# CraigIDent/SpliSER

Measured on AMD Instinct MI355X. Metric: splice sites/sec (+ reads/sec) processed, higher is better.
Workload: dtype int32/u32 counters, f64 SSE

## Files before the change

spliser_amd/csrc/spl_device.h:

```cpp
#ifndef SPL_DEVICE_H
#define SPL_DEVICE_H

#include <stdint.h>
#include <hip/hip_vector_types.h>

#include "spl_pack.h"
#include "spl_devpack.h"

#ifndef SPL_BLOCK
#define SPL_BLOCK 256
#endif
#define SPL_COUNTER_STRIDE 64
#define SPL_WAVES (SPL_BLOCK / 64)
#ifndef SPL_K_SIMPLE
#define SPL_K_SIMPLE 4
#define SPL_K_MNM 2
#endif
#ifndef SPL_LIST_K
#define SPL_LIST_K 2
#endif
#ifndef SPL_WAVE_ITERS
#define SPL_WAVE_ITERS 10
#endif
#define SPL_WAVE_READS (64 * SPL_WAVE_ITERS)
#define SPL_TILE_FUSED_SHIFT 10
#define SPL_TILE_FUSED (1 << SPL_TILE_FUSED_SHIFT)
#define SPL_BLOCK_FUSED 256
#define SPL_WAVE_READS_FUSED 512
#define SPL_WIN 1020
#define SPL_WIN_STRANDED 956
#define SPL_WIN_STRANDED_FUSED 508
#define SPL_SERIAL_MAX 8
#ifndef SPL_AGG_ROUNDS
#define SPL_AGG_ROUNDS 2
#endif
#define SPL_LITERAL_WAVES 8192
#ifndef SPL_SCAN_BLOCK
#define SPL_SCAN_BLOCK 256
#endif


#define SPL_DEV_ERR_RANGE 1
#define SPL_DEV_ERR_TABLE 2

#define SPL_JF_COUNT_MASK 0x00ffffffu
#define SPL_JF_COMPLEX 0x40000000u
#define SPL_JF_MULTIROW 0x80000000u

#define SPL_SF_PLUS 1u
#define SPL_SF_MINUS 2u

struct spl_dbk {
    uint32_t first;
    uint32_t occ;
    uint32_t rival;
};

struct spl_count_params {
    int64_t n_reads;
    uint32_t n_chunks;
    const spl_chunk_meta *chunk_meta;
// ... 127 lines not shown
```

spliser_amd/csrc/spl_kernels.hip:

```cpp
#include <hip/hip_runtime.h>
#include <hip/hip_ext.h>
#include <cstdio>
#include <cstdlib>
#include <stdint.h>

#define SPL_HD __device__ __forceinline__
#include "spl_classify.h"
#include "spl_device.h"
#include "spl_layout_tile.h"

namespace {

__device__ __forceinline__ int32_t first_site_at_or_after(const spl_count_params &p, int32_t pos)
{
    const int64_t rel = (int64_t)pos - (int64_t)p.bucket_base;
    uint32_t b = 0;
    if (rel > 0) {
        const int64_t q = rel >> p.bucket_shift;
        b = q >= (int64_t)p.n_buckets ? p.n_buckets : (uint32_t)q;
    }
    uint32_t lo = p.bucket[b];
    uint32_t hi = p.bucket[b < p.n_buckets ? b + 1 : b];
    while (lo < hi) {
        const uint32_t mid = (lo + hi) >> 1;
// ... 328 lines not shown
    rv = (e.rival >> ((uint32_t)(x - p.dbase) & 31u)) & 1u;
}

typedef __attribute__((address_space(3))) int32_t spl_lds_i32;

template <int NARR, int WIN = (NARR == 4 ? SPL_WIN_STRANDED : SPL_WIN)>
__device__ __forceinline__ void commit_key(const spl_hot_params &p, spl_lds_i32 *lds, int32_t wbase, bool valid, uint32_t key, int32_t sign)
{
    if (valid) {
        const int arr = (int)(key & 3u);
        const int32_t d = (int32_t)(key >> 2);
        const uint32_t loc = (uint32_t)(d - wbase);
        if (loc <= (uint32_t)WIN) __hip_atomic_fetch_add(lds + (arr * (WIN + 1) + (int)loc), sign, __ATOMIC_RELAXED, __HIP_MEMORY_SCOPE_WORKGROUP);
        else atomicAdd(&p.diff[(int64_t)arr * p.diff_stride + d], sign);
    }
}

template <int NARR, int WIN>
__device__ __forceinline__ void commit_range(const spl_hot_params &p, spl_lds_i32 *lds, int32_t wbase, bool em, int32_t lo, int32_t ub, uint32_t arr)
{
    const uint32_t a = (uint32_t)(lo - wbase), b = (uint32_t)(ub - wbase);
    const bool inside = a <= (uint32_t)WIN && b <= (uint32_t)WIN;
    if (em && inside) {
        spl_lds_i32 *const row = lds + (int)arr * (WIN + 1);
        __hip_atomic_fetch_add(row + (int)a, 1, __ATOMIC_RELAXED, __HIP_MEMORY_SCOPE_WORKGROUP);
        __hip_atomic_fetch_add(row + (int)b, -1, __ATOMIC_RELAXED, __HIP_MEMORY_SCOPE_WORKGROUP);
    }
    if (__any(em && !inside)) {
        commit_key<NARR, WIN>(p, lds, wbase, em && !inside, ((uint32_t)lo << 2) | arr, 1);
        commit_key<NARR, WIN>(p, lds, wbase, em && !inside, ((uint32_t)ub << 2) | arr, -1);
    }
}

__device__ __forceinline__ void agg_add(uint32_t *addr, int32_t delta)
{
    const int lane = (int)__builtin_amdgcn_mbcnt_hi(~0u, __builtin_amdgcn_mbcnt_lo(~0u, 0u));
    unsigned long long todo = __ballot(1);
    const uint32_t lo = (uint32_t)(uintptr_t)addr, hi = (uint32_t)((uintptr_t)addr >> 32);
    for (int round = 0; round < SPL_AGG_ROUNDS; ++round) {
        const int leader = __ffsll((long long)todo) - 1;
        const bool same = (__shfl((int)lo, leader) == (int)lo) && (__shfl((int)hi, leader) == (int)hi);
        const unsigned long long grp = __ballot(same);
        const unsigned long long plus = __ballot(same && delta > 0);
        if (lane == leader) {
            const int32_t sum = 2 * (int32_t)__popcll(plus) - (int32_t)__popcll(grp);
            if (sum) atomicAdd(addr, (uint32_t)sum);
        }
        if (same) return;
        todo &= ~grp;
    }
    atomicAdd(addr, (uint32_t)delta);
}


__device__ __forceinline__ uint32_t junction_hash(int32_t l, int32_t r)
{
    uint32_t h = (uint32_t)l * 0x9E3779B1u ^ (uint32_t)r * 0x85EBCA77u;
    return h ^ (h >> 15);
}

template <bool STRANDED, int NARR, int WIN = (NARR == 4 ? SPL_WIN_STRANDED : SPL_WIN)>
__device__ __forceinline__ bool rivals_inline_from(const spl_hot_params &p, spl_lds_i32 *lds, int32_t wbase, int32_t l, int32_t r, uint32_t h,
                                                   uint4 ent, uint4 first, const int32_t *blk_a, const int32_t *blk_b, uint32_t sidx)
{
    bool found = false;
    for (int probe = 0; probe < 8; ++probe) {
// ... 92 lines not shown
                if (t > jl[a] && t < jr[a]) inside = a;
                if (jl[a] == t) { pu = jr[a]; alpha = true; }
                if (jr[a] == t) { pu = jl[a]; alpha = true; }
            }
#pragma unroll
            for (int b = 0; b < 3; ++b) cov |= (blk_a[b] <= t) && (t + 1 <= blk_b[b]);
            const bool beta1type = !alpha && inside < 0 && cov && strand_ok;
            if (alpha || beta1type) {
                const uint4 rx = p.jrivals[2u * (r_off[j] + i) + 1u];
                for (uint32_t e2 = 0; e2 < rx.z; ++e2) {
                    const int32_t pp = p.part_pos[rx.y + e2];
                    const bool is_end = pp == jl[0] || pp == jr[0] || pp == jl[1] || pp == jr[1];
                    if (is_end && !(alpha && pp == pu)) agg_add(&p.dbl[rx.y + e2], 1);
                }
                if (beta1type) {
                    commit_key<NARR, WIN>(p, lds, wbase, true, (td << 2) | a_b1, -1);
                    commit_key<NARR, WIN>(p, lds, wbase, true, ((td + 1u) << 2) | a_b1, 1);
                    commit_key<NARR, WIN>(p, lds, wbase, true, (td << 2) | a_me, 1);
                    commit_key<NARR, WIN>(p, lds, wbase, true, ((td + 1u) << 2) | a_me, -1);
                }
            } else if (inside >= j && strand_ok) {
                commit_key<NARR, WIN>(p, lds, wbase, true, (td << 2) | a_me, -1);
                commit_key<NARR, WIN>(p, lds, wbase, true, ((td + 1u) << 2) | a_me, 1);
            }
        }
    }
    return true;
}

}


template <bool STRANDED, bool BIG, bool FUSED>
__global__ __launch_bounds__(FUSED ? SPL_BLOCK_FUSED : SPL_BLOCK) __attribute__((amdgpu_waves_per_eu(FUSED ? 4 : 8, 8))) void spl_count_ranges_kernel(const spl_hot_params p)
{
    constexpr int NARR = STRANDED ? 4 : 2;
    constexpr int WIN = STRANDED ? (FUSED ? SPL_WIN_STRANDED_FUSED : SPL_WIN_STRANDED) : SPL_WIN;
    __shared__ int32_t lds_words[NARR * (WIN + 1)];
    spl_lds_i32 *const lds = (spl_lds_i32 *)lds_words;
    constexpr int BLOCK = FUSED ? SPL_BLOCK_FUSED : SPL_BLOCK, NWAVE = BLOCK / 64;
    constexpr int RPT = (int)SPL_TILE_FUSED / SPL_BLOCK_FUSED;
    constexpr uint32_t SEG = FUSED ? SPL_WAVE_READS_FUSED : SPL_WAVE_READS;
    constexpr uint32_t CSHIFT = BIG ? SPL_CHUNK_BIG_SHIFT : SPL_CHUNK_SHIFT;
    constexpr uint32_t TILE = SPL_TILE_FUSED, TILES = FUSED ? (1u << CSHIFT) / TILE : 1u;
    constexpr uint32_t REC_BYTES = FUSED ? (uint32_t)SPL_LAYOUT_SLOT(TILE) : 16u;
    __shared__ uint4 s_rec[REC_BYTES / 16u];
    __shared__ uint16_t s_idx[FUSED ? TILE : 1];
    __shared__ uint32_t s_lay[2 * NWAVE];
    typedef __attribute__((address_space(3))) const char spl_lchar;
    spl_lchar *const lrec = (spl_lchar *)s_rec;
    __shared__ uint16_t s_q[NWAVE * SEG];
    __shared__ uint32_t s_qcnt[NWAVE], s_qbase;
    const uint32_t wave = (uint32_t)__builtin_amdgcn_readfirstlane((int)(threadIdx.x >> 6));
    const uint32_t seg0 = wave * SEG;
    const uint32_t lane = (uint32_t)threadIdx.x & 63u;
    uint32_t n_front = 0, n_back = 0, back_done = 0;
    uint32_t fm_mnm = 0, it_mnm = 0;
    auto rank_in = [](unsigned long long m) {
        return (uint32_t)__builtin_amdgcn_mbcnt_hi((uint32_t)(m >> 32), __builtin_amdgcn_mbcnt_lo((uint32_t)m, 0u));
    };
    const uint32_t chunk_slot = my_chunk();
    const uint32_t ordered = chunk_slot < p.n_chunks ? p.chunk_order[chunk_slot] : 0xffffffffu;
    const bool live = ordered != 0xffffffffu;
    const uint32_t chunk = live ? ordered : 0u;
    uint32_t n_simple = 0;
    auto entry_of = [&](uint32_t slot) { return FUSED ? (uint32_t)((__attribute__((address_space(3))) const uint16_t *)s_idx)[(slot & 0x3fffu) - n_simple] : slot; };
    auto push_direct = [&](bool want, uint32_t slot, unsigned long long m, uint32_t n) {
        const uint32_t shard = blockIdx.x & 7u;
        uint32_t base = 0;
        if (lane == 0) base = atomicAdd(&p.queue_n[shard * SPL_COUNTER_STRIDE], n);
        base = (uint32_t)__builtin_amdgcn_readfirstlane((int)base);
        if (want) p.queue[(size_t)shard * p.queue_cap + base + rank_in(m)] = (chunk << CSHIFT) | entry_of(slot);
    };
    auto push_front = [&](bool want, uint32_t slot) {
        const unsigned long long m = __ballot(want);
        const uint32_t n = (uint32_t)__popcll(m);
        if (n_front + n_back - back_done + n > SEG) { push_direct(want, slot, m, n); return; }
        if (want) s_q[seg0 + n_front + rank_in(m)] = (uint16_t)entry_of(slot);
        n_front += n;
    };
    auto push_back = [&](bool want, uint32_t slot) {
        const unsigned long long m = __ballot(want);
        const uint32_t n = (uint32_t)__popcll(m);
        if (n_front + n_back + n > SEG) { push_front(want, slot & 0x3fffu); return; }
        if (want) s_q[seg0 + SEG - 1u - n_back - rank_in(m)] = (uint16_t)slot;
        n_back += n;
    };

    const int tid = threadIdx.x;
    int32_t wbase = 0;
    ChunkView cv;
    typedef __attribute__((address_space(1))) const uint32_t spl_gdw;
    auto dbk_at = [&](uint32_t s) { return (spl_gdw *)((__attribute__((address_space(1))) const char *)p.dbucket + (size_t)((s << 3) + (s << 2))); };
    auto dbk2 = [&](uint32_t s) { spl_gdw *q = dbk_at(s); spl_dbk e; e.first = q[0]; e.occ = q[1]; e.rival = 0u; return e; };
    auto dbk3 = [&](uint32_t s) { spl_gdw *q = dbk_at(s); spl_dbk e; e.first = q[0]; e.occ = q[1]; e.rival = q[2]; return e; };
    spl_layout_chunk ch;
    uint32_t tile = 0, tile_last = 0;
    uint32_t ob[TILES + 1];
    auto span_of = [&](uint32_t k) {
        const int64_t g0 = ch.lo & ~(int64_t)((1u << CSHIFT) - 1u), hi = ch.lo + ch.n;
        spllay::TileSpan sp;
        sp.cell0 = g0 + (int64_t)k * TILE;
        sp.lo = sp.cell0 > ch.lo ? sp.cell0 : ch.lo;
        sp.hi = sp.cell0 + TILE < hi ? sp.cell0 + TILE : hi;
        uint32_t a = ob[0], b = ob[1];
#pragma unroll
        for (uint32_t q = 1; q < TILES; ++q) { a = k == q ? ob[q] : a; b = k == q ? ob[q + 1] : b; }
        sp.o_lo = a; sp.o_hi = b; sp.o_fetch_hi = ch.o_hi; sp.seg_op0 = ch.seg_op0;
        return sp;
    };
    if constexpr (FUSED) {
        if (!live) return;
        ch = p.cells[chunk];
        const int64_t g0 = ch.lo & ~(int64_t)((1u << CSHIFT) - 1u), hi = ch.lo + ch.n;
        tile = (uint32_t)((ch.lo - g0) >> SPL_TILE_FUSED_SHIFT);
        tile_last = (uint32_t)((hi - 1 - g0) >> SPL_TILE_FUSED_SHIFT);
        const int32_t fp0 = p.src.pos[ch.lo] + ch.shift;
        const spl_dbk e_first = p.dbucket[dbk_slot(p, fp0 - 1)];
#pragma unroll
        for (uint32_t q = 0; q <= TILES; ++q) {
            int64_t i = g0 + (int64_t)q * TILE;
            i = i < ch.lo ? ch.lo : (i > hi ? hi : i);
            ob[q] = q == 0u ? ch.o_lo : (q == TILES ? ch.o_hi : p.src.cig_off[i]);
        }
        for (int j = tid; j < NARR * (WIN + 1); j += BLOCK) lds[j] = 0;
        cv.rec = nullptr;
        cv.wide = (spl_gu32 *)(p.src.cigar + ch.seg_op0);
        cv.shift = ch.shift;
        cv.first_pos = fp0 - ch.shift;
        { uint32_t nv; dbk_resolve(p, fp0 - 1, e_first, wbase, nv); }
    } else {
        cv = chunk_view(p.chunk_meta + chunk);
    }
    typedef uint32_t u32x4_a8 __attribute__((ext_vector_type(4), aligned(8)));
    auto ld_r4 = [&](uint32_t at) {
        if constexpr (FUSED) { const u32x4_a8 v = *(__attribute__((address_space(3))) const u32x4_a8 *)(lrec + at); return make_uint4(v.x, v.y, v.z, v.w); }
        else return ld_g4(cv.rec + (size_t)at);
    };
    auto ld_r2 = [&](uint32_t at) {
        if constexpr (FUSED) { const spl_u32x2 v = *(__attribute__((address_space(3))) const spl_u32x2 *)(lrec + at); return make_uint2(v.x, v.y); }
        else return ld_g2(cv.rec + (size_t)at);
    };
    for (;;) {
    if constexpr (FUSED) {
        const spllay::TileSpan sp = span_of(tile);
        uint32_t n[4];
        {
            spllay::TileLoads<(int)TILE, RPT> L;
            spllay::tile_issue<(int)TILE, RPT>(p.src, p.src_n_rec, p.src_n_ops, sp, L);
            spllay::tile_finish<(int)TILE, RPT>(p.src, p.src_n_ops, sp, L, (spllay::lay_lds_w32 *)s_rec, (spllay::lay_lds_w32 *)s_lay,
                                                spllay::RecordsInLds{(spllay::lay_lds_u8 *)s_rec, (spllay::lay_lds_u16 *)s_idx, tile * TILE}, n);
        }
        cv.start[0] = 0; cv.start[1] = n[0]; cv.start[2] = n[0] + n[1]; cv.start[3] = n[0] + n[1] + n[2]; cv.start[4] = n[0] + n[1] + n[2] + n[3];
        cv.off[0] = 0;
        cv.off[1] = (n[0] * SPL_REC_SIMPLE + 15u) & ~15u;
        cv.off[2] = cv.off[1] + n[1] * SPL_REC_MNM;
        cv.off[3] = cv.off[2] + n[2] * SPL_REC_M2;
        n_simple = n[0];
        __syncthreads();
    }
    constexpr uint32_t KS = SPL_K_SIMPLE, KM = SPL_K_MNM;
    uint32_t g_start[SPL_RC_RUNS + 1];
    g_start[0] = 0;
    g_start[1] = (cv.start[1] + 64u * KS - 1u) / (64u * KS);
    g_start[2] = g_start[1] + (cv.start[2] - cv.start[1] + 64u * KM - 1u) / (64u * KM);
    g_start[3] = g_start[2] + ((cv.start[3] - cv.start[2] + 63u) >> 6);
    g_start[4] = g_start[3] + ((cv.start[4] - cv.start[3] + 63u) >> 6);
    const uint32_t g_total = live ? g_start[SPL_RC_RUNS] : 0u;
    typedef uint4 W4;
    W4 cu0 = make_uint4(0, 0, 0, 0), cu1 = make_uint4(0, 0, 0, 0);
    uint32_t cu_i0 = 0;
    auto fetch = [&](uint32_t g) {
        const uint32_t run = (g >= g_start[1] ? 1u : 0u) + (g >= g_start[2] ? 1u : 0u) + (g >= g_start[3] ? 1u : 0u);
        uint32_t gs = 0, n_run = cv.start[1], off = 0, size = SPL_REC_SIMPLE, per = KS;
        if (run == 1u) { gs = g_start[1]; n_run = cv.start[2] - cv.start[1]; off = cv.off[1]; size = SPL_REC_MNM; per = KM; }
        if (run == 2u) { gs = g_start[2]; n_run = cv.start[3] - cv.start[2]; off = cv.off[2]; size = SPL_REC_M2; per = 1u; }
        if (run == 3u) { gs = g_start[3]; n_run = cv.start[4] - cv.start[3]; off = cv.off[3]; size = SPL_REC_OTHER; per = 1u; }
        const uint32_t i0 = (((g - gs) << 6) + lane) * per;

        cu_i0 = i0;
        const uint32_t r = off + (i0 < n_run ? i0 : 0u) * size;
        cu0 = ld_r4(r);
        cu1 = ld_r4(r + 16u);
    };
    if constexpr (!FUSED) { if (wave < g_total) fetch(wave); }
    if constexpr (!FUSED) {
        { const int32_t fp = cv.first_pos + cv.shift; uint32_t nv; const spl_dbk e = p.dbucket[dbk_slot(p, fp - 1)]; dbk_resolve(p, fp - 1, e, wbase, nv); }
        for (int j = tid; j < NARR * (WIN + 1); j += BLOCK) lds[j] = 0;
        __syncthreads();
    }

    {
        uint32_t g = live ? wave : g_start[SPL_RC_RUNS];
        auto fetch_next = [&]() { if constexpr (!FUSED) fetch(g + NWAVE < g_total ? g + NWAVE : g); };
        auto take = [&](uint32_t gs, uint32_t n_run, uint32_t off, uint32_t size, uint32_t per) {
            if constexpr (FUSED) {
                const uint32_t i0 = (((g - gs) << 6) + lane) * per;
                cu_i0 = i0;
                const uint32_t r = off + (i0 < n_run ? i0 : 0u) * size;
                cu0 = ld_r4(r);
                cu1 = ld_r4(r + 16u);
            }
        };
        for (; g < g_start[1]; g += NWAVE) {
            take(0u, cv.start[1], 0u, SPL_REC_SIMPLE, KS);
            const uint32_t i0 = cu_i0;
            const W4 r0 = cu0, r1 = cu1;
            const uint32_t n_run = cv.start[1];
            const uint32_t w[8] = {r0.x, r0.y, r0.z, r0.w, r1.x, r1.y, r1.z, r1.w};
            int32_t pos[KS], c1[KS];
            spl_dbk e0[KS], e1[KS];
#pragma unroll
            for (uint32_t j = 0; j < KS; ++j) {
                pos[j] = (int32_t)w[2 * j] + cv.shift;
                c1[j] = pos[j] + (int32_t)(w[2 * j + 1] >> 16);
                e0[j] = dbk2(dbk_slot(p, pos[j] - 1));
                e1[j] = dbk2(dbk_slot(p, c1[j] - 1));
            }
            fetch_next();
#pragma unroll
            for (uint32_t j = 0; j < KS; ++j) {
                int32_t ua, ub; uint32_t nva, nvb;
                dbk_resolve(p, pos[j] - 1, e0[j], ua, nva);
                dbk_resolve(p, c1[j] - 1, e1[j], ub, nvb);
                const int32_t lo = ua + (int32_t)nva;
                const bool emit = i0 + j < n_run && ub > lo;
                uint32_t arr = 0;
                if (STRANDED) arr = (spl_read_strand(w[2 * j + 1] & 0xffffu, p.stranded) == (uint8_t)'-') ? 1u : 0u;
                if (__any(emit)) commit_range<NARR, WIN>(p, lds, wbase, emit, lo, ub, arr);
            }
        }
        for (; g < g_start[2]; g += NWAVE) {
            take(g_start[1], cv.start[2] - cv.start[1], cv.off[1], SPL_REC_MNM, KM);
            const uint32_t i0 = cu_i0;
            const W4 r0 = cu0, r1 = cu1;
            const uint32_t n_run = cv.start[2] - cv.start[1];
// ... 209 lines not shown
                bool live[KM], undecided[KM];
                int32_t pos[KM], c0[KM], c1[KM], c2[KM];
                uint32_t h[KM];
                uint4 ent[KM], first[KM];
#pragma unroll
                for (uint32_t k = 0; k < KM; ++k) {
                    live[k] = ((bits >> k) & 1u) != 0u;
                    undecided[k] = false;
                    pos[k] = (int32_t)w[4 * k] + cv.shift;
                    c0[k] = pos[k] + (int32_t)(w[4 * k + 1] >> 16); c1[k] = c0[k] + (int32_t)w[4 * k + 2]; c2[k] = c1[k] + (int32_t)w[4 * k + 3];
                    h[k] = junction_hash(c0[k] - 1, c1[k] - 1);
                    ent[k] = first[k] = make_uint4(0x80000000u, 0u, 0u, 0u);
                    if (live[k]) {
                        const uint4 *hslot = p.jhash + 2u * (h[k] & p.jhash_mask);
                        ent[k] = hslot[0];
                        first[k] = hslot[1];
                    }
                }
#pragma unroll
                for (uint32_t k = 0; k < KM; ++k) {
                    uint32_t sidx = 0;
                    if (STRANDED) sidx = (spl_read_strand(w[4 * k + 1] & 0xffffu, p.stranded) == (uint8_t)'-') ? 1u : 0u;
                    const int32_t blk_a[2] = {pos[k], c1[k]}, blk_b[2] = {c0[k] - 1, c2[k] - 1};
                    if (live[k]) undecided[k] = !rivals_inline_from<STRANDED, NARR, WIN>(p, lds, wbase, c0[k] - 1, c1[k] - 1, h[k], ent[k], first[k], blk_a, blk_b, sidx);
                }
#pragma unroll
                for (uint32_t k = 0; k < KM; ++k)
                    if (__any(undecided[k])) push_front(undecided[k], cv.start[1] + i0 + k);
            }
        }
    }
    if constexpr (!FUSED) break;
    else {
        if (tile == tile_last) break;
        ++tile;
        fm_mnm = 0; it_mnm = 0; n_back = 0; back_done = 0;
        __syncthreads();
    }
    }
    if ((tid & 63) == 0) s_qcnt[tid >> 6] = n_front;
    __syncthreads();
    uint32_t q_start[NWAVE + 1];
    q_start[0] = 0;
#pragma unroll
    for (int w = 0; w < NWAVE; ++w) q_start[w + 1] = q_start[w] + s_qcnt[w];
    const uint32_t qn = q_start[NWAVE];
    if (qn) {
        const uint32_t shard = blockIdx.x & 7u;
        if (tid == 0) s_qbase = atomicAdd(&p.queue_n[shard * SPL_COUNTER_STRIDE], qn);
        __syncthreads();
        uint32_t *dst = p.queue + (size_t)shard * p.queue_cap + s_qbase;
        const uint32_t first = chunk << CSHIFT;
        for (uint32_t j = tid; j < qn; j += BLOCK) {
            uint32_t w = 0;
#pragma unroll
            for (int k = 1; k < NWAVE; ++k) w += (j >= q_start[k]) ? 1u : 0u;
            uint32_t base = 0;
#pragma unroll
            for (int k = 0; k < NWAVE; ++k) base = (w == (uint32_t)k) ? q_start[k] : base;
            dst[j] = first | (uint32_t)s_q[w * SEG + (j - base)];
        }
    }
    for (int j = tid; j < NARR * (WIN + 1); j += BLOCK) {
        const int32_t v = lds[j];
        if (v) {
            const int arr = j / (WIN + 1), loc = j - arr * (WIN + 1);
            atomicAdd(&p.diff[(int64_t)arr * p.diff_stride + wbase + loc], v);
        }
    }
}

namespace {
// ... 474 lines not shown
                       n_dpos, flag_pos, n_flag, dbase, n_dbuckets, out);
    return (int)hipGetLastError();
}

extern "C" int spl_dev_launch_clear(void *region, size_t bytes, void *stream)
{
    const size_t n16 = bytes / 16;
    size_t blocks = (n16 + 256 * 4 - 1) / (256 * 4);
    blocks = blocks < 1 ? 1 : (blocks > 4096 ? 4096 : blocks);
    hipLaunchKernelGGL(spl_clear_kernel, dim3((uint32_t)blocks), dim3(256), 0, (hipStream_t)stream, (uint4 *)region, n16);
    return (int)hipGetLastError();
}

extern "C" int spl_dev_launch_count(const spl_count_params *p, const spl_hot_params *h, int pairs, void *stream, int *grid_out, int *lds_out,
                                    void *ev_start, void *ev_stop)
{
    *grid_out = 0;
    *lds_out = 0;
    if (p->n_reads <= 0 || p->n_sites <= 0) return 0;
    const uint32_t slots = pairs ? ((p->n_chunks + 7u) / 8u) * 8u : h->n_chunks;
    const uint32_t grid = slots;
    *grid_out = (int)grid;
    hipStream_t st = (hipStream_t)stream;
    hipEvent_t e0 = (hipEvent_t)ev_start, e1 = (hipEvent_t)ev_stop;
    if (pairs) {
        *lds_out = 2 * SPL_WIN * 4 + SPL_BLOCK * 5 * 4 + 4;
        if (p->stranded) hipExtLaunchKernelGGL(spl_count_pairs_kernel<true>, dim3(grid), dim3(SPL_BLOCK), 0, st, e0, e1, 0, *p);
        else hipExtLaunchKernelGGL(spl_count_pairs_kernel<false>, dim3(grid), dim3(SPL_BLOCK), 0, st, e0, e1, 0, *p);
    } else {
        const bool big = h->chunk_shift == SPL_CHUNK_BIG_SHIFT;
        *lds_out = (p->stranded ? 4 * ((h->cells ? SPL_WIN_STRANDED_FUSED : SPL_WIN_STRANDED) + 1) : 2 * (SPL_WIN + 1)) * 4 + SPL_WAVES * SPL_WAVE_READS * 2 + 4 * SPL_WAVES + 4;
#define SPL_LAUNCH_RANGES(S, B) hipExtLaunchKernelGGL((spl_count_ranges_kernel<S, B, false>), dim3(grid), dim3(SPL_BLOCK), 0, st, e0, e1, 0, *h)
        if (h->cells) {
            *lds_out += (int)SPL_LAYOUT_SLOT(SPL_TILE_FUSED) + 2 * SPL_TILE_FUSED + (SPL_BLOCK_FUSED / 64) * SPL_WAVE_READS_FUSED * 2 - SPL_WAVES * SPL_WAVE_READS * 2;
#define SPL_LAUNCH_FUSED(S, B) hipExtLaunchKernelGGL((spl_count_ranges_kernel<S, B, true>), dim3(grid), dim3(SPL_BLOCK_FUSED), 0, st, e0, e1, 0, *h)
            if (p->stranded) { if (big) SPL_LAUNCH_FUSED(true, true); else SPL_LAUNCH_FUSED(true, false); }
            else { if (big) SPL_LAUNCH_FUSED(false, true); else SPL_LAUNCH_FUSED(false, false); }
#undef SPL_LAUNCH_FUSED
        } else if (p->stranded) {
            if (big) SPL_LAUNCH_RANGES(true, true); else SPL_LAUNCH_RANGES(true, false);
        } else {
            if (big) SPL_LAUNCH_RANGES(false, true); else SPL_LAUNCH_RANGES(false, false);
        }
#undef SPL_LAUNCH_RANGES
    }
    return (int)hipGetLastError();
}

extern "C" int spl_dev_launch_literal(const spl_count_params *p, const spl_queue_params *q, void *stream)
{
    if (p->n_reads <= 0 || p->n_sites <= 0) return 0;
    hipStream_t st = (hipStream_t)stream;
    const uint32_t grid = SPL_LITERAL_WAVES;
    if (p->stranded) hipLaunchKernelGGL(spl_count_literal_kernel<true>, dim3(grid), dim3(64), 0, st, *p, *q);
    else hipLaunchKernelGGL(spl_count_literal_kernel<false>, dim3(grid), dim3(64), 0, st, *p, *q);
    return (int)hipGetLastError();
}

extern "C" int spl_dev_launch_scan(const spl_scan_params *p, void *stream)
{
    if (p->n_dpos <= 0) return 0;
    hipStream_t st = (hipStream_t)stream;
    hipLaunchKernelGGL(spl_scan_apply_kernel, dim3(p->n_blocks), dim3(256), 0, st, *p);
    return (int)hipGetLastError();
}

extern "C" int spl_dev_launch_sse(const spl_sse_params *p, void *stream)
// ... 7 lines not shown
```

spliser_amd/csrc/spl_layout_tile.h:

```cpp
#ifndef SPL_LAYOUT_TILE_H
#define SPL_LAYOUT_TILE_H
#include <hip/hip_runtime.h>
#include <stdint.h>

#include "spl_pack.h"
#include "spl_devpack.h"

namespace spllay {

typedef uint32_t lay_u32x2 __attribute__((ext_vector_type(2)));
typedef uint32_t lay_u32x4 __attribute__((ext_vector_type(4)));
typedef lay_u32x2 lay_u32x2_a4 __attribute__((aligned(4)));
typedef lay_u32x4 lay_u32x4_a8 __attribute__((aligned(8)));
typedef __attribute__((address_space(3))) uint32_t lay_lds_w32;
typedef __attribute__((address_space(3))) int32_t lay_lds_i32;
typedef __attribute__((address_space(3))) uint8_t lay_lds_u8;
typedef __attribute__((address_space(3))) uint16_t lay_lds_u16;

typedef __attribute__((address_space(3))) const uint32_t lay_lds_u32;
struct StagedOps {
    static constexpr bool padded = true;
    lay_lds_u32 *p;
    __device__ __forceinline__ uint32_t operator()(uint32_t k) const { return p[k]; }
};
__device__ __forceinline__ uint32_t row_scan(uint32_t v)
{
    v += (uint32_t)__builtin_amdgcn_update_dpp(0, (int)v, 0x111, 0xf, 0xf, false);
    v += (uint32_t)__builtin_amdgcn_update_dpp(0, (int)v, 0x112, 0xf, 0xf, false);
    v += (uint32_t)__builtin_amdgcn_update_dpp(0, (int)v, 0x114, 0xf, 0xf, false);
    v += (uint32_t)__builtin_amdgcn_update_dpp(0, (int)v, 0x118, 0xf, 0xf, false);
    return v;
}

__device__ __forceinline__ uint32_t wave_scan(uint32_t v)
{
    v += (uint32_t)__builtin_amdgcn_update_dpp(0, (int)v, 0x111, 0xf, 0xf, false);
    v += (uint32_t)__builtin_amdgcn_update_dpp(0, (int)v, 0x112, 0xf, 0xf, false);
    v += (uint32_t)__builtin_amdgcn_update_dpp(0, (int)v, 0x114, 0xf, 0xf, false);
    v += (uint32_t)__builtin_amdgcn_update_dpp(0, (int)v, 0x118, 0xf, 0xf, false);
    v += (uint32_t)__builtin_amdgcn_update_dpp(0, (int)v, 0x142, 0xa, 0xf, false);
    v += (uint32_t)__builtin_amdgcn_update_dpp(0, (int)v, 0x143, 0xc, 0xf, false);
    return v;
}


struct RecordsInMemory {
    static constexpr bool wants_index = false;
    static constexpr bool clip_tier = false;
    uint8_t *rec_base;
    size_t slot_bytes;
    __device__ __forceinline__ uint8_t *rec() const { return rec_base + (size_t)blockIdx.x * slot_bytes; }
    __device__ __forceinline__ void st2(uint32_t d, lay_u32x2 v) const { *(lay_u32x2 *)(rec() + d) = v; }
    __device__ __forceinline__ void st4(uint32_t d, lay_u32x4 v) const { *(lay_u32x4_a8 *)(rec() + d) = v; }
    __device__ __forceinline__ void index(uint32_t, uint32_t) const {}
};
struct RecordsInLds {
    static constexpr bool wants_index = true;
    static constexpr bool clip_tier = true;
    lay_lds_u8 *rec;
    lay_lds_u16 *idx;
    uint32_t base;
    __device__ __forceinline__ void st2(uint32_t d, lay_u32x2 v) const { *(__attribute__((address_space(3))) lay_u32x2 *)(rec + d) = v; }
    __device__ __forceinline__ void st4(uint32_t d, lay_u32x4 v) const { *(__attribute__((address_space(3))) lay_u32x4_a8 *)(rec + d) = v; }
    __device__ __forceinline__ void index(uint32_t q, uint32_t cell_index) const { idx[q] = (uint16_t)(base + cell_index); }
};

struct TileSpan { int64_t cell0, lo, hi; uint32_t o_lo, o_hi, o_fetch_hi, seg_op0; };
template <int C, int R>
struct TileLoads {
    int32_t pos[R];
    uint32_t fw[R / 2];
    uint32_t co[R + 1];
    lay_u32x4 v[R];
};

template <int C, int R>
__device__ __forceinline__ void tile_issue(const spl_devreads &src, int64_t n_rec, int64_t n_ops, const TileSpan &sp, TileLoads<C, R> &L)
{
    static_assert(R == 4 || R == 2, "two or four reads a thread");
    constexpr uint32_t T = C / R, STAGE = 4 * C;
    static_assert(STAGE / (4 * T) == R, "R quads of ops a thread");
    const uint32_t t = threadIdx.x;
    const int64_t g = sp.cell0 + R * (int64_t)t;
#pragma unroll
    for (int j = 0; j < R; ++j) L.pos[j] = 0;
#pragma unroll
    for (int j = 0; j <= R; ++j) L.co[j] = 0;
#pragma unroll
    for (int j = 0; j < R / 2; ++j) L.fw[j] = 0;
    const uint32_t r0 = (uint32_t)R * t, lo_r = (uint32_t)(sp.lo - sp.cell0), hi_r = (uint32_t)(sp.hi - sp.cell0);
    const int64_t left = n_rec - sp.cell0;
    const uint32_t rec_r = left < (int64_t)C ? (uint32_t)left : (uint32_t)C;
    const bool mine = r0 + R > lo_r && r0 < hi_r;
    if (mine) {
        if (r0 + R <= rec_r) {
            if constexpr (R == 4) {
                const lay_u32x4 pv = *(const lay_u32x4 *)(src.pos + g);
                const lay_u32x2 fv = *(const lay_u32x2 *)(src.flag + g);
                const lay_u32x4 cv = *(const lay_u32x4 *)(src.cig_off + g);
                L.co[4] = src.cig_off[g + 4];
                L.pos[0] = (int32_t)pv.x; L.pos[1] = (int32_t)pv.y; L.pos[2] = (int32_t)pv.z; L.pos[3] = (int32_t)pv.w;
                L.fw[0] = fv.x; L.fw[1] = fv.y;
                L.co[0] = cv.x; L.co[1] = cv.y; L.co[2] = cv.z; L.co[3] = cv.w;
            } else {
                const lay_u32x2 pv = *(const lay_u32x2 *)(src.pos + g);
                L.fw[0] = *(const uint32_t *)(src.flag + g);
                const lay_u32x2 cv = *(const lay_u32x2 *)(src.cig_off + g);
                L.co[2] = src.cig_off[g + 2];
                L.pos[0] = (int32_t)pv.x; L.pos[1] = (int32_t)pv.y;
                L.co[0] = cv.x; L.co[1] = cv.y;
            }
        } else {
            uint32_t f[R];
#pragma unroll
            for (int j = 0; j < R; ++j) {
                const int64_t i = g + j;
                f[j] = 0;
                if (i < n_rec) { L.pos[j] = src.pos[i]; f[j] = src.flag[i]; L.co[j] = src.cig_off[i]; L.co[j + 1] = src.cig_off[i + 1]; }
                else L.co[j + 1] = L.co[j];
            }
#pragma unroll
            for (int j = 0; j < R / 2; ++j) L.fw[j] = f[2 * j] | (f[2 * j + 1] << 16);
        }
    }
    const uint64_t ws = sp.o_lo & ~3u;
    const uint64_t o_end = (uint64_t)sp.o_fetch_hi < ws + STAGE ? (uint64_t)sp.o_fetch_hi : ws + STAGE;
#pragma unroll
    for (uint32_t q = 0; q < (uint32_t)R; ++q) {
        const uint64_t at = ws + 4ull * (t + q * T);
        L.v[q] = lay_u32x4{0u, 0u, 0u, 0u};
        if (at < o_end) {
            if (at + 4 <= (uint64_t)n_ops) L.v[q] = *(const lay_u32x4 *)(src.cigar + at);
            else {
                L.v[q].x = src.cigar[at];
                if (at + 1 < (uint64_t)n_ops) L.v[q].y = src.cigar[at + 1];
                if (at + 2 < (uint64_t)n_ops) L.v[q].z = src.cigar[at + 2];
            }
        }
    }
}

template <int C, int R, class Sink>
__device__ __forceinline__ void tile_finish(const spl_devreads &src, int64_t n_ops, const TileSpan &sp, const TileLoads<C, R> &L, lay_lds_w32 *s_ops,
                                            lay_lds_w32 *s_cnt, const Sink sink, uint32_t (&n)[4])
{
    constexpr uint32_t T = C / R, NW = T / 64, STAGE = 4 * C;
    static_assert(NW <= 16, "the waves' totals are summed inside one row of lanes");
    constexpr uint32_t PAD = SPL_PACK_SCAN_OPS;
    const uint32_t t = threadIdx.x, lane = t & 63u, wave = t >> 6;
    const int64_t g = sp.cell0 + R * (int64_t)t;
    const uint32_t r0 = (uint32_t)R * t, lo_r = (uint32_t)(sp.lo - sp.cell0), hi_r = (uint32_t)(sp.hi - sp.cell0);
    const uint32_t o_hi = sp.o_hi, seg_op0 = sp.seg_op0;
    int32_t pos[R];
    uint32_t flag[R], co[R + 1];
#pragma unroll
    for (int j = 0; j < R; ++j) { pos[j] = L.pos[j]; flag[j] = (j & 1) ? L.fw[j / 2] >> 16 : L.fw[j / 2] & 0xffffu; }
#pragma unroll
    for (int j = 0; j <= R; ++j) co[j] = L.co[j];
    auto fill = [&](uint64_t ws) {
        const uint64_t o_end = (uint64_t)o_hi < ws + STAGE ? (uint64_t)o_hi : ws + STAGE;
        lay_u32x4 v[R];
#pragma unroll
        for (uint32_t q = 0; q < (uint32_t)R; ++q) {
            const uint64_t at = ws + 4ull * (t + q * T);
            v[q] = lay_u32x4{0u, 0u, 0u, 0u};
            if (at < o_end) {
                if (at + 4 <= (uint64_t)n_ops) v[q] = *(const lay_u32x4 *)(src.cigar + at);
                else {
                    v[q].x = src.cigar[at];
                    if (at + 1 < (uint64_t)n_ops) v[q].y = src.cigar[at + 1];
                    if (at + 2 < (uint64_t)n_ops) v[q].z = src.cigar[at + 2];
                }
            }
        }
#pragma unroll
        for (uint32_t q = 0; q < (uint32_t)R; ++q) *(__attribute__((address_space(3))) lay_u32x4 *)(s_ops + 4u * (t + q * T)) = v[q];
    };
    uint64_t ws = sp.o_lo & ~3u;
#pragma unroll
    for (uint32_t q = 0; q < (uint32_t)R; ++q) *(__attribute__((address_space(3))) lay_u32x4 *)(s_ops + 4u * (t + q * T)) = L.v[q];
    __syncthreads();

// ... 29 lines not shown
            for (int q = 0; q < 6; ++q) w[j][q] = take ? r.w[q] : w[j][q];
            __builtin_amdgcn_sched_barrier(0);
        }
    }
    for (;;) {
        if (__any(pend != 0u)) {
#pragma unroll
            for (int j = 0; j < R; ++j) {
                if ((pend >> j) & 1u) {
                    const uint32_t c0 = src.cig_off[g + j], c1 = src.cig_off[g + j + 1], rel0 = c0 - (uint32_t)ws;
                    if (rel0 + PAD <= STAGE) {
                        splrec::Rec r;
                        splrec::classify_lean((int32_t)w[j][0], w[j][1] & 0xffffu, StagedOps{(lay_lds_u32 *)s_ops + rel0}, c1 - c0, c0 - seg_op0, r);
                        runs = (runs & ~(7u << (3 * j))) | (r.run << (3 * j));
                        pend &= ~(1u << j);
#pragma unroll
                        for (int q = 0; q < 6; ++q) w[j][q] = r.w[q];
                    }
                }
                __builtin_amdgcn_sched_barrier(0);
            }
        }
        if (ws + STAGE >= (uint64_t)o_hi + PAD) break;
        ws += STAGE - PAD;
        __syncthreads();
        fill(ws);
        __syncthreads();
    }
    uint32_t c01 = 0, c23 = 0;
    uint32_t run[R];
#pragma unroll
    for (int j = 0; j < R; ++j) {
        run[j] = (runs >> (3 * j)) & 7u;
        c01 += run[j] == SPL_RC_SIMPLE ? 1u : (run[j] == SPL_RC_MNM ? 0x10000u : 0u);
        c23 += run[j] == SPL_RC_M2 ? 1u : (run[j] == SPL_RC_OTHER ? 0x10000u : 0u);
    }

    const uint32_t i01 = wave_scan(c01), i23 = wave_scan(c23);
    if (lane == 63u) { s_cnt[2u * wave] = i01; s_cnt[2u * wave + 1u] = i23; }
    __syncthreads();
    const uint32_t x = row_scan(lane < NW ? s_cnt[2u * (lane < NW ? lane : 0u)] : 0u), y = row_scan(lane < NW ? s_cnt[2u * (lane < NW ? lane : 0u) + 1u] : 0u);
    const uint32_t wu = (uint32_t)__builtin_amdgcn_readfirstlane((int)wave);
    const uint32_t t01 = (uint32_t)__builtin_amdgcn_readlane((int)x, NW - 1), t23 = (uint32_t)__builtin_amdgcn_readlane((int)y, NW - 1);
    const uint32_t b01 = wu ? (uint32_t)__builtin_amdgcn_readlane((int)x, wu - 1u) : 0u, b23 = wu ? (uint32_t)__builtin_amdgcn_readlane((int)y, wu - 1u) : 0u;
    const uint32_t n0 = t01 & 0xffffu, n1 = t01 >> 16, n2 = t23 & 0xffffu, n3 = t23 >> 16;
    const uint32_t off1 = (n0 * SPL_REC_SIMPLE + 15u) & ~15u, off2 = off1 + n1 * SPL_REC_MNM, off3 = off2 + n2 * SPL_REC_M2;
    const uint32_t e01 = b01 + i01 - c01, e23 = b23 + i23 - c23;
    uint32_t at[4] = {(e01 & 0xffffu) * SPL_REC_SIMPLE, off1 + (e01 >> 16) * SPL_REC_MNM, off2 + (e23 & 0xffffu) * SPL_REC_M2, off3 + (e23 >> 16) * SPL_REC_OTHER};
    [[maybe_unused]] uint32_t q_at[3] = {e01 >> 16, n1 + (e23 & 0xffffu), n1 + n2 + (e23 >> 16)};

#pragma unroll
    for (int j = 0; j < R; ++j) {
        const uint32_t r = run[j];
        const uint32_t d = r == SPL_RC_SIMPLE ? at[0] : (r == SPL_RC_MNM ? at[1] : (r == SPL_RC_M2 ? at[2] : at[3]));
        if (r == SPL_RC_SIMPLE) sink.st2(d, lay_u32x2{w[j][0], w[j][1]});
        else if (r < (uint32_t)SPL_RC_RUNS) {
            sink.st4(d, lay_u32x4{w[j][0], w[j][1], w[j][2], w[j][3]});
            if (r != SPL_RC_MNM) sink.st2(d + 16, lay_u32x2{w[j][4], w[j][5]});
            if constexpr (Sink::wants_index) {
                sink.index(r == SPL_RC_MNM ? q_at[0] : (r == SPL_RC_M2 ? q_at[1] : q_at[2]), (uint32_t)R * t + (uint32_t)j);
                q_at[0] += r == SPL_RC_MNM ? 1u : 0u;
                q_at[1] += r == SPL_RC_M2 ? 1u : 0u;
                q_at[2] += r == SPL_RC_OTHER ? 1u : 0u;
            }
        }
        at[0] += r == SPL_RC_SIMPLE ? SPL_REC_SIMPLE : 0u;
        at[1] += r == SPL_RC_MNM ? SPL_REC_MNM : 0u;
        at[2] += r == SPL_RC_M2 ? SPL_REC_M2 : 0u;
        at[3] += r == SPL_RC_OTHER ? SPL_REC_OTHER : 0u;
    }
    n[0] = n0; n[1] = n1; n[2] = n2; n[3] = n3;
}

template <int C, class Sink>
__device__ __forceinline__ void layout_tile(const spl_devreads &src, int64_t n_rec, int64_t n_ops, const spl_layout_chunk &ch, lay_lds_w32 *s_ops,
                                            lay_lds_w32 *s_cnt, lay_lds_i32 *s_first, const Sink sink, uint32_t (&n)[4])
{
    const TileSpan sp{ch.lo & ~(int64_t)(C - 1), ch.lo, ch.lo + ch.n, ch.o_lo, ch.o_hi, ch.o_hi, ch.seg_op0};
    TileLoads<C, 4> L;
    tile_issue<C, 4>(src, n_rec, n_ops, sp, L);
    const int64_t g = sp.cell0 + 4 * (int64_t)threadIdx.x;
    if (sp.lo >= g && sp.lo < g + 4) {
        const uint32_t e = (uint32_t)(sp.lo - g);
        *s_first = e == 0u ? L.pos[0] : (e == 1u ? L.pos[1] : (e == 2u ? L.pos[2] : L.pos[3]));
    }
    tile_finish<C, 4>(src, n_ops, sp, L, s_ops, s_cnt, sink, n);
}

}
#endif
```

Measured before the change: 159.4 million.

## Commit simple reads in place during tile layout instead of staging them in LDS

In the fused count kernel, simple (single-junction) reads are now resolved and committed to the LDS difference arrays directly inside tile_finish, rather than being written as records to shared memory and re-read by a separate per-wave loop. That loop is disabled for the fused path. The record buffer is shrunk to a fixed size, so a tile whose remaining records overflow it is reprocessed as two half-tiles. The waves-per-EU hint rises from 4 to 5 to use the freed LDS for occupancy. The gains are less LDS traffic and higher occupancy. The costs are more register pressure in tile_finish and a possible second pass over overflowing tiles.

```diff
diff --git a/spliser_amd/csrc/spl_device.h b/spliser_amd/csrc/spl_device.h
--- a/spliser_amd/csrc/spl_device.h
+++ b/spliser_amd/csrc/spl_device.h
@@ -27,6 +27,7 @@
 #define SPL_TILE_FUSED (1 << SPL_TILE_FUSED_SHIFT)
 #define SPL_BLOCK_FUSED 256
 #define SPL_WAVE_READS_FUSED 512
+#define SPL_REC_BYTES_FUSED 16448
 #define SPL_WIN 1020
 #define SPL_WIN_STRANDED 956
 #define SPL_WIN_STRANDED_FUSED 508
diff --git a/spliser_amd/csrc/spl_kernels.hip b/spliser_amd/csrc/spl_kernels.hip
--- a/spliser_amd/csrc/spl_kernels.hip
+++ b/spliser_amd/csrc/spl_kernels.hip
@@ -384,6 +384,47 @@
     }
 }
 
+__device__ __forceinline__ spl_dbk dbk_load2(const spl_hot_params &p, uint32_t s)
+{
+    typedef __attribute__((address_space(1))) const uint32_t gdw;
+    gdw *q = (gdw *)((__attribute__((address_space(1))) const char *)p.dbucket + (size_t)((s << 3) + (s << 2)));
+    spl_dbk e; e.first = q[0]; e.occ = q[1]; e.rival = 0u;
+    return e;
+}
+
+template <bool STRANDED, int NARR, int WIN, int R>
+struct SimpleInPlace {
+    static constexpr bool in_place = true;
+    const spl_hot_params &p;
+    spl_lds_i32 *lds;
+    int32_t wbase, shift;
+    bool active;
+    spl_dbk e0[R], e1[R];
+    __device__ __forceinline__ void issue(int j, bool is_simple, uint32_t w0, uint32_t w1)
+    {
+        if (!active || !__any(is_simple)) return;
+        const int32_t a = (int32_t)w0 + shift, b = a + (int32_t)(w1 >> 16);
+        e0[j] = e1[j] = spl_dbk{0u, 0u, 0u};
+        if (is_simple) {
+            e0[j] = dbk_load2(p, dbk_slot(p, a - 1));
+            e1[j] = dbk_load2(p, dbk_slot(p, b - 1));
+        }
+    }
+    __device__ __forceinline__ void commit(int j, bool is_simple, uint32_t w0, uint32_t w1)
+    {
+        if (!active || !__any(is_simple)) return;
+        const int32_t a = (int32_t)w0 + shift, b = a + (int32_t)(w1 >> 16);
+        int32_t ua, ub; uint32_t nva, nvb;
+        dbk_resolve(p, a - 1, e0[j], ua, nva);
+        dbk_resolve(p, b - 1, e1[j], ub, nvb);
+        const int32_t lo = ua + (int32_t)nva;
+        const bool emit = is_simple && ub > lo;
+        uint32_t arr = 0;
+        if (STRANDED) arr = (spl_read_strand(w1 & 0xffffu, p.stranded) == (uint8_t)'-') ? 1u : 0u;
+        if (__any(emit)) commit_range<NARR, WIN>(p, lds, wbase, emit, lo, ub, arr);
+    }
+};
+
 __device__ __forceinline__ void agg_add(uint32_t *addr, int32_t delta)
 {
     const int lane = (int)__builtin_amdgcn_mbcnt_hi(~0u, __builtin_amdgcn_mbcnt_lo(~0u, 0u));
@@ -542,7 +583,7 @@
 
 
 template <bool STRANDED, bool BIG, bool FUSED>
-__global__ __launch_bounds__(FUSED ? SPL_BLOCK_FUSED : SPL_BLOCK) __attribute__((amdgpu_waves_per_eu(FUSED ? 4 : 8, 8))) void spl_count_ranges_kernel(const spl_hot_params p)
+__global__ __launch_bounds__(FUSED ? SPL_BLOCK_FUSED : SPL_BLOCK) __attribute__((amdgpu_waves_per_eu(FUSED ? 5 : 8, 8))) void spl_count_ranges_kernel(const spl_hot_params p)
 {
     constexpr int NARR = STRANDED ? 4 : 2;
     constexpr int WIN = STRANDED ? (FUSED ? SPL_WIN_STRANDED_FUSED : SPL_WIN_STRANDED) : SPL_WIN;
@@ -553,7 +594,8 @@
     constexpr uint32_t SEG = FUSED ? SPL_WAVE_READS_FUSED : SPL_WAVE_READS;
     constexpr uint32_t CSHIFT = BIG ? SPL_CHUNK_BIG_SHIFT : SPL_CHUNK_SHIFT;
     constexpr uint32_t TILE = SPL_TILE_FUSED, TILES = FUSED ? (1u << CSHIFT) / TILE : 1u;
-    constexpr uint32_t REC_BYTES = FUSED ? (uint32_t)SPL_LAYOUT_SLOT(TILE) : 16u;
+    constexpr uint32_t REC_BYTES = FUSED ? (uint32_t)SPL_REC_BYTES_FUSED : 16u, REC_ROOM = REC_BYTES - 64u;
+    static_assert(!FUSED || (REC_ROOM >= 16u * TILE && REC_ROOM >= (TILE / 2u) * SPL_REC_OTHER), "a tile's ops, and half a tile's records whatever they are");
     __shared__ uint4 s_rec[REC_BYTES / 16u];
     __shared__ uint16_t s_idx[FUSED ? TILE : 1];
     __shared__ uint32_t s_lay[2 * NWAVE];
@@ -563,7 +605,7 @@
     __shared__ uint32_t s_qcnt[NWAVE], s_qbase;
     const uint32_t wave = (uint32_t)__builtin_amdgcn_readfirstlane((int)(threadIdx.x >> 6));
     const uint32_t seg0 = wave * SEG;
-    const uint32_t lane = (uint32_t)threadIdx.x & 63u;
+    uint32_t lane = (uint32_t)threadIdx.x & 63u;
     uint32_t n_front = 0, n_back = 0, back_done = 0;
     uint32_t fm_mnm = 0, it_mnm = 0;
     auto rank_in = [](unsigned long long m) {
@@ -573,8 +615,7 @@
     const uint32_t ordered = chunk_slot < p.n_chunks ? p.chunk_order[chunk_slot] : 0xffffffffu;
     const bool live = ordered != 0xffffffffu;
     const uint32_t chunk = live ? ordered : 0u;
-    uint32_t n_simple = 0;
-    auto entry_of = [&](uint32_t slot) { return FUSED ? (uint32_t)((__attribute__((address_space(3))) const uint16_t *)s_idx)[(slot & 0x3fffu) - n_simple] : slot; };
+    auto entry_of = [&](uint32_t slot) { return FUSED ? (uint32_t)((__attribute__((address_space(3))) const uint16_t *)s_idx)[slot & 0x3fffu] : slot; };
     auto push_direct = [&](bool want, uint32_t slot, unsigned long long m, uint32_t n) {
         const uint32_t shard = blockIdx.x & 7u;
         uint32_t base = 0;
@@ -597,7 +638,7 @@
         n_back += n;
     };
 
-    const int tid = threadIdx.x;
+    int tid = threadIdx.x;
     int32_t wbase = 0;
     ChunkView cv;
     typedef __attribute__((address_space(1))) const uint32_t spl_gdw;
@@ -651,22 +692,32 @@
         if constexpr (FUSED) { const spl_u32x2 v = *(__attribute__((address_space(3))) const spl_u32x2 *)(lrec + at); return make_uint2(v.x, v.y); }
         else return ld_g2(cv.rec + (size_t)at);
     };
+    uint32_t half = 0;
     for (;;) {
     if constexpr (FUSED) {
-        const spllay::TileSpan sp = span_of(tile);
-        uint32_t n[4];
-        {
+        lane = spllay::thread_here() & 63u;
+        spllay::TileSpan sp = span_of(tile);
+        if (half) {
+            int64_t mid = sp.cell0 + (int64_t)(TILE / 2u);
+            mid = mid < sp.lo ? sp.lo : (mid > sp.hi ? sp.hi : mid);
+            const uint32_t o_mid = p.src.cig_off[mid];
+            if (half == 1u) { sp.hi = mid; sp.o_hi = o_mid; } else { sp.lo = mid; sp.o_lo = o_mid; }
+        }
+        uint32_t n[4] = {0, 0, 0, 0};
+        bool fits = true;
+        if (sp.hi > sp.lo) {
+            SimpleInPlace<STRANDED, NARR, WIN, RPT> simple{p, lds, wbase, ch.shift, half == 0u};
             spllay::TileLoads<(int)TILE, RPT> L;
             spllay::tile_issue<(int)TILE, RPT>(p.src, p.src_n_rec, p.src_n_ops, sp, L);
-            spllay::tile_finish<(int)TILE, RPT>(p.src, p.src_n_ops, sp, L, (spllay::lay_lds_w32 *)s_rec, (spllay::lay_lds_w32 *)s_lay,
-                                                spllay::RecordsInLds{(spllay::lay_lds_u8 *)s_rec, (spllay::lay_lds_u16 *)s_idx, tile * TILE}, n);
-        }
-        cv.start[0] = 0; cv.start[1] = n[0]; cv.start[2] = n[0] + n[1]; cv.start[3] = n[0] + n[1] + n[2]; cv.start[4] = n[0] + n[1] + n[2] + n[3];
+            fits = spllay::tile_finish<(int)TILE, RPT>(p.src, p.src_n_ops, sp, L, (spllay::lay_lds_w32 *)s_rec, (spllay::lay_lds_w32 *)s_lay,
+                                                       spllay::RecordsInLds{(spllay::lay_lds_u8 *)s_rec, (spllay::lay_lds_u16 *)s_idx, tile * TILE}, simple, n, REC_ROOM);
+        }
+        if (!fits) { half = 1u; continue; }
+        cv.start[0] = 0; cv.start[1] = 0; cv.start[2] = n[1]; cv.start[3] = n[1] + n[2]; cv.start[4] = n[1] + n[2] + n[3];
         cv.off[0] = 0;
-        cv.off[1] = (n[0] * SPL_REC_SIMPLE + 15u) & ~15u;
-        cv.off[2] = cv.off[1] + n[1] * SPL_REC_MNM;
+        cv.off[1] = 0;
+        cv.off[2] = n[1] * SPL_REC_MNM;
         cv.off[3] = cv.off[2] + n[2] * SPL_REC_M2;
-        n_simple = n[0];
         __syncthreads();
     }
     constexpr uint32_t KS = SPL_K_SIMPLE, KM = SPL_K_MNM;
@@ -712,6 +763,7 @@
                 cu1 = ld_r4(r + 16u);
             }
         };
+        if constexpr (!FUSED)
         for (; g < g_start[1]; g += NWAVE) {
             take(0u, cv.start[1], 0u, SPL_REC_SIMPLE, KS);
             const uint32_t i0 = cu_i0;
@@ -987,12 +1039,17 @@
     }
     if constexpr (!FUSED) break;
     else {
-        if (tile == tile_last) break;
-        ++tile;
+        if (half == 1u) half = 2u;
+        else {
+            if (tile == tile_last) break;
+            ++tile;
+            half = 0u;
+        }
         fm_mnm = 0; it_mnm = 0; n_back = 0; back_done = 0;
         __syncthreads();
     }
     }
+    if constexpr (FUSED) tid = (int)spllay::thread_here();
     if ((tid & 63) == 0) s_qcnt[tid >> 6] = n_front;
     __syncthreads();
     uint32_t q_start[NWAVE + 1];
@@ -1533,7 +1590,7 @@
         *lds_out = (p->stranded ? 4 * ((h->cells ? SPL_WIN_STRANDED_FUSED : SPL_WIN_STRANDED) + 1) : 2 * (SPL_WIN + 1)) * 4 + SPL_WAVES * SPL_WAVE_READS * 2 + 4 * SPL_WAVES + 4;
 #define SPL_LAUNCH_RANGES(S, B) hipExtLaunchKernelGGL((spl_count_ranges_kernel<S, B, false>), dim3(grid), dim3(SPL_BLOCK), 0, st, e0, e1, 0, *h)
         if (h->cells) {
-            *lds_out += (int)SPL_LAYOUT_SLOT(SPL_TILE_FUSED) + 2 * SPL_TILE_FUSED + (SPL_BLOCK_FUSED / 64) * SPL_WAVE_READS_FUSED * 2 - SPL_WAVES * SPL_WAVE_READS * 2;
+            *lds_out += (int)SPL_REC_BYTES_FUSED + 2 * SPL_TILE_FUSED + (SPL_BLOCK_FUSED / 64) * SPL_WAVE_READS_FUSED * 2 - SPL_WAVES * SPL_WAVE_READS * 2;
 #define SPL_LAUNCH_FUSED(S, B) hipExtLaunchKernelGGL((spl_count_ranges_kernel<S, B, true>), dim3(grid), dim3(SPL_BLOCK_FUSED), 0, st, e0, e1, 0, *h)
             if (p->stranded) { if (big) SPL_LAUNCH_FUSED(true, true); else SPL_LAUNCH_FUSED(true, false); }
             else { if (big) SPL_LAUNCH_FUSED(false, true); else SPL_LAUNCH_FUSED(false, false); }
diff --git a/spliser_amd/csrc/spl_layout_tile.h b/spliser_amd/csrc/spl_layout_tile.h
--- a/spliser_amd/csrc/spl_layout_tile.h
+++ b/spliser_amd/csrc/spl_layout_tile.h
@@ -23,6 +23,12 @@
     lay_lds_u32 *p;
     __device__ __forceinline__ uint32_t operator()(uint32_t k) const { return p[k]; }
 };
+__device__ __forceinline__ uint32_t thread_here()
+{
+    uint32_t t = threadIdx.x;
+    asm volatile("" : "+v"(t));
+    return t;
+}
 __device__ __forceinline__ uint32_t row_scan(uint32_t v)
 {
     v += (uint32_t)__builtin_amdgcn_update_dpp(0, (int)v, 0x111, 0xf, 0xf, false);
@@ -64,6 +70,7 @@
     __device__ __forceinline__ void st4(uint32_t d, lay_u32x4 v) const { *(__attribute__((address_space(3))) lay_u32x4_a8 *)(rec + d) = v; }
     __device__ __forceinline__ void index(uint32_t q, uint32_t cell_index) const { idx[q] = (uint16_t)(base + cell_index); }
 };
+struct SimpleAsRecords { static constexpr bool in_place = false; };
 
 struct TileSpan { int64_t cell0, lo, hi; uint32_t o_lo, o_hi, o_fetch_hi, seg_op0; };
 template <int C, int R>
@@ -80,7 +87,7 @@
     static_assert(R == 4 || R == 2, "two or four reads a thread");
     constexpr uint32_t T = C / R, STAGE = 4 * C;
     static_assert(STAGE / (4 * T) == R, "R quads of ops a thread");
-    const uint32_t t = threadIdx.x;
+    const uint32_t t = thread_here();
     const int64_t g = sp.cell0 + R * (int64_t)t;
 #pragma unroll
     for (int j = 0; j < R; ++j) L.pos[j] = 0;
@@ -140,14 +147,14 @@
     }
 }
 
-template <int C, int R, class Sink>
-__device__ __forceinline__ void tile_finish(const spl_devreads &src, int64_t n_ops, const TileSpan &sp, const TileLoads<C, R> &L, lay_lds_w32 *s_ops,
-                                            lay_lds_w32 *s_cnt, const Sink sink, uint32_t (&n)[4])
+template <int C, int R, class Sink, class Simple>
+__device__ __forceinline__ bool tile_finish(const spl_devreads &src, int64_t n_ops, const TileSpan &sp, const TileLoads<C, R> &L, lay_lds_w32 *s_ops,
+                                            lay_lds_w32 *s_cnt, const Sink sink, Simple &simple, uint32_t (&n)[4], uint32_t room = 0xffffffffu)
 {
     constexpr uint32_t T = C / R, NW = T / 64, STAGE = 4 * C;
     static_assert(NW <= 16, "the waves' totals are summed inside one row of lanes");
     constexpr uint32_t PAD = SPL_PACK_SCAN_OPS;
-    const uint32_t t = threadIdx.x, lane = t & 63u, wave = t >> 6;
+    const uint32_t t = thread_here(), lane = t & 63u, wave = t >> 6;
     const int64_t g = sp.cell0 + R * (int64_t)t;
     const uint32_t r0 = (uint32_t)R * t, lo_r = (uint32_t)(sp.lo - sp.cell0), hi_r = (uint32_t)(sp.hi - sp.cell0);
     const uint32_t o_hi = sp.o_hi, seg_op0 = sp.seg_op0;
@@ -243,6 +250,10 @@
 #pragma unroll
     for (int j = 0; j < R; ++j) {
         run[j] = (runs >> (3 * j)) & 7u;
+        if constexpr (Simple::in_place) {
+            simple.issue(j, run[j] == SPL_RC_SIMPLE, w[j][0], w[j][1]);
+            c01 += run[j] == SPL_RC_MNM ? 0x10000u : 0u;
+        } else
         c01 += run[j] == SPL_RC_SIMPLE ? 1u : (run[j] == SPL_RC_MNM ? 0x10000u : 0u);
         c23 += run[j] == SPL_RC_M2 ? 1u : (run[j] == SPL_RC_OTHER ? 0x10000u : 0u);
     }
@@ -256,6 +267,14 @@
     const uint32_t b01 = wu ? (uint32_t)__builtin_amdgcn_readlane((int)x, wu - 1u) : 0u, b23 = wu ? (uint32_t)__builtin_amdgcn_readlane((int)y, wu - 1u) : 0u;
     const uint32_t n0 = t01 & 0xffffu, n1 = t01 >> 16, n2 = t23 & 0xffffu, n3 = t23 >> 16;
     const uint32_t off1 = (n0 * SPL_REC_SIMPLE + 15u) & ~15u, off2 = off1 + n1 * SPL_REC_MNM, off3 = off2 + n2 * SPL_REC_M2;
+    n[0] = n0; n[1] = n1; n[2] = n2; n[3] = n3;
+    if (off3 + n3 * SPL_REC_OTHER > room) {
+        if constexpr (Simple::in_place) {
+#pragma unroll
+            for (int j = 0; j < R; ++j) simple.commit(j, run[j] == SPL_RC_SIMPLE, w[j][0], w[j][1]);
+        }
+        return false;
+    }
     const uint32_t e01 = b01 + i01 - c01, e23 = b23 + i23 - c23;
     uint32_t at[4] = {(e01 & 0xffffu) * SPL_REC_SIMPLE, off1 + (e01 >> 16) * SPL_REC_MNM, off2 + (e23 & 0xffffu) * SPL_REC_M2, off3 + (e23 >> 16) * SPL_REC_OTHER};
     [[maybe_unused]] uint32_t q_at[3] = {e01 >> 16, n1 + (e23 & 0xffffu), n1 + n2 + (e23 >> 16)};
@@ -263,8 +282,9 @@
 #pragma unroll
     for (int j = 0; j < R; ++j) {
         const uint32_t r = run[j];
-        const uint32_t d = r == SPL_RC_SIMPLE ? at[0] : (r == SPL_RC_MNM ? at[1] : (r == SPL_RC_M2 ? at[2] : at[3]));
-        if (r == SPL_RC_SIMPLE) sink.st2(d, lay_u32x2{w[j][0], w[j][1]});
+        uint32_t d = r == SPL_RC_MNM ? at[1] : (r == SPL_RC_M2 ? at[2] : at[3]);
+        if constexpr (!Simple::in_place) d = r == SPL_RC_SIMPLE ? at[0] : d;
+        if (r == SPL_RC_SIMPLE) { if constexpr (!Simple::in_place) sink.st2(d, lay_u32x2{w[j][0], w[j][1]}); }
         else if (r < (uint32_t)SPL_RC_RUNS) {
             sink.st4(d, lay_u32x4{w[j][0], w[j][1], w[j][2], w[j][3]});
             if (r != SPL_RC_MNM) sink.st2(d + 16, lay_u32x2{w[j][4], w[j][5]});
@@ -275,12 +295,16 @@
                 q_at[2] += r == SPL_RC_OTHER ? 1u : 0u;
             }
         }
-        at[0] += r == SPL_RC_SIMPLE ? SPL_REC_SIMPLE : 0u;
+        if constexpr (!Simple::in_place) at[0] += r == SPL_RC_SIMPLE ? SPL_REC_SIMPLE : 0u;
         at[1] += r == SPL_RC_MNM ? SPL_REC_MNM : 0u;
         at[2] += r == SPL_RC_M2 ? SPL_REC_M2 : 0u;
         at[3] += r == SPL_RC_OTHER ? SPL_REC_OTHER : 0u;
     }
-    n[0] = n0; n[1] = n1; n[2] = n2; n[3] = n3;
+    if constexpr (Simple::in_place) {
+#pragma unroll
+        for (int j = 0; j < R; ++j) simple.commit(j, run[j] == SPL_RC_SIMPLE, w[j][0], w[j][1]);
+    }
+    return true;
 }
 
 template <int C, class Sink>
@@ -295,7 +319,8 @@
         const uint32_t e = (uint32_t)(sp.lo - g);
         *s_first = e == 0u ? L.pos[0] : (e == 1u ? L.pos[1] : (e == 2u ? L.pos[2] : L.pos[3]));
     }
-    tile_finish<C, 4>(src, n_ops, sp, L, s_ops, s_cnt, sink, n);
+    SimpleAsRecords as_records;
+    (void)tile_finish<C, 4>(src, n_ops, sp, L, s_ops, s_cnt, sink, as_records, n);
 }
 
 }
```

Measured after the change: 164.2 million, median of 6. 3.1% higher.
